# HarrisonKramer/optiland

Hardware: AMD Instinct MI355X
Metric: ray-surface intersections/s (higher is better)
Workload: dtype f32

## Files before the change

### optiland_amd/csrc/trace_kernel.hip

```cpp
#include <hip/hip_runtime.h>
#include <stdint.h>
#include <math.h>
#include <stdlib.h>

#include <type_traits>

#include "device_table.h"
#include "raygen_device.h"
#include "wavefront_device.h"
#include "epilogue_device.h"
#include "trace_launch.h"

#ifndef OL_TABLE_IN_LDS
#define OL_TABLE_IN_LDS 0
#endif
#ifndef OL_NR_PREFETCH
#define OL_NR_PREFETCH 0
#endif
#ifndef OL_PREFETCH_F64
#define OL_PREFETCH_F64 1
#endif
#ifndef OL_FUSED_NR_PREFETCH
#define OL_FUSED_NR_PREFETCH 1
#endif
#ifndef OL_FETCH_NR_F32
#define OL_FETCH_NR_F32 0
#endif
#ifndef OL_FETCH_NR_F32_PLAIN
#define OL_FETCH_NR_F32_PLAIN 1
#endif
#ifndef OL_FETCH_NR_F64
#define OL_FETCH_NR_F64 2
#endif
#ifndef OL_FETCH_NR_F64_ASPHERE
#define OL_FETCH_NR_F64_ASPHERE 1
#endif
#ifndef OL_FETCH_LEAN_F64
#define OL_FETCH_LEAN_F64 1
#endif
#ifndef OL_FETCH_LEAN_F32
#define OL_FETCH_LEAN_F32 1
#endif

#include "surface_math.h"

namespace ol {

template <typename T, int NR, bool FUSED, int POLK = 0>
constexpr int fetch_level() {
  if (OL_TABLE_IN_LDS) return 0;
  if (NR != 0) {
    if (sizeof(T) == 4) return (!FUSED && POLK == 0) ? OL_FETCH_NR_F32_PLAIN : OL_FETCH_NR_F32;
    return NR == kNrEvenAsphere ? OL_FETCH_NR_F64_ASPHERE : OL_FETCH_NR_F64;
  }
  if (!FUSED) return 0;
  return sizeof(T) == 4 ? OL_FETCH_LEAN_F32 : OL_FETCH_LEAN_F64;
}

template <typename T, int RPT, int POLK, int NR>
struct LanePack {
#ifndef OL_PACKED_F32
#define OL_PACKED_F32 1
#endif
#ifndef OL_POLZ_PACKED
#define OL_POLZ_PACKED 1
#endif
  static constexpr bool packed =
      sizeof(T) == 4 && ((OL_PACKED_F32 && (RPT == 4 || RPT == 2) && POLK == 0 && NR == 0) ||
                         (OL_POLZ_PACKED && RPT == 2 && POLK == 1 && NR == kNrZernike));
  using V = typename std::conditional<packed, f32x2, T>::type;
  static constexpr int NV = packed ? RPT / 2 : RPT;
  using PT = typename PrtLane<V, POLK>::type;
  using PrtArr = Prt<PT, POLK>[POLK ? NV : 1];
  static __device__ __forceinline__ T pget(const PrtArr& P, int k, int e) {
    if constexpr (packed && POLK != 0) return P[k / 2].m[e][k % 2]; else return P[k].m[e];
  }
  static __device__ __forceinline__ void pset(PrtArr& P, int k, int e, T x) {
    if constexpr (packed && POLK != 0) P[k / 2].m[e][k % 2] = x; else P[k].m[e] = x;
  }
  static __device__ __forceinline__ T get(const V& v, int e) {
    if constexpr (packed) return v[e]; else return v;
  }
  static __device__ __forceinline__ void set(V& v, int e, T x) {
    if constexpr (packed) v[e] = x; else v = x;
  }
  static __device__ __forceinline__ Ray<T> ray(const Ray<V> (&r)[NV], int k) {
    constexpr int L = packed ? 2 : 1;
    const Ray<V>& p = r[k / L];
    const int e = k % L;
    Ray<T> o;
    o.x = get(p.x, e); o.y = get(p.y, e); o.z = get(p.z, e);
    o.L = get(p.L, e); o.M = get(p.M, e); o.N = get(p.N, e);
    o.i = get(p.i, e); o.opd = get(p.opd, e);
    return o;
  }
  static __device__ __forceinline__ void put(Ray<V> (&r)[NV], int k, const Ray<T>& o) {
    constexpr int L = packed ? 2 : 1;
    Ray<V>& p = r[k / L];
    const int e = k % L;
    set(p.x, e, o.x); set(p.y, e, o.y); set(p.z, e, o.z);
    set(p.L, e, o.L); set(p.M, e, o.M); set(p.N, e, o.N);
    set(p.i, e, o.i); set(p.opd, e, o.opd);
  }
};

#ifndef OL_NT_SCALAR
#define OL_NT_SCALAR 1
#endif
#ifndef OL_NT_VECTOR
#define OL_NT_VECTOR 0
#endif

template <typename T, int RPT>
struct VecOf {
  typedef T type __attribute__((ext_vector_type(RPT)));
};

template <typename T, int RPT>
__device__ __forceinline__ T vec_get(const typename VecOf<T, RPT>::type& v, int k) {
  return v[k];
}

#ifndef OL_SADDR
#define OL_SADDR 1
#endif
#ifndef OL_RECORD_DIRECT
#define OL_RECORD_DIRECT 0
#endif
#ifndef OL_RECORD_ARGS_FRESH
#define OL_RECORD_ARGS_FRESH 1
#endif
#ifndef OL_PRT_SCALAR_BASE
#define OL_PRT_SCALAR_BASE 0
#endif
template <bool SADDR>
struct RayIndexT {
  int64_t tile;
  uint32_t lane;
  __device__ __forceinline__ int64_t full() const { return tile + (int64_t)lane; }
  template <typename P>
  __device__ __forceinline__ P* at(P* p) const {
    if constexpr (SADDR)
      return (p + tile) + lane;
    else
      return p + (tile + (int64_t)lane);
  }
};

template <typename T, int RPT, typename RayIndex>
__device__ __forceinline__ void store_plane(T* __restrict__ p, RayIndex base, int cnt,
                                            const T (&in)[RPT]) {
  T* q = base.at(p);
  if constexpr (RPT == 1) {
#if OL_NT_SCALAR
    __builtin_nontemporal_store(in[0], q);
#else
    *q = in[0];
#endif
  } else {
    using V = typename VecOf<T, RPT>::type;
    if (cnt == RPT) {
      V v;
#pragma unroll
      for (int k = 0; k < RPT; ++k) v[k] = in[k];
      if constexpr (OL_NT_VECTOR || sizeof(V) <= 8)
        __builtin_nontemporal_store(v, reinterpret_cast<V*>(q));
      else
        *reinterpret_cast<V*>(q) = v;
    } else {
#pragma unroll
      for (int k = 0; k < RPT; ++k)
        if (k < cnt) q[k] = in[k];
    }
  }
}

template <typename T, int RPT, typename RayIndex>
__device__ __forceinline__ void store_rays(T* __restrict__ row, int64_t stride, RayIndex base,
                                           int cnt, const Ray<T> (&g)[RPT]) {
  T tmp[RPT];
#define OL_STORE_FIELD(idx, fld)                         \
  _Pragma("unroll") for (int k = 0; k < RPT; ++k) tmp[k] = g[k].fld; \
  store_plane<T, RPT>(row + (int64_t)(idx) * stride, base, cnt, tmp);
  OL_STORE_FIELD(0, x)
  OL_STORE_FIELD(1, y)
  OL_STORE_FIELD(2, z)
  OL_STORE_FIELD(3, L)
  OL_STORE_FIELD(4, M)
  OL_STORE_FIELD(5, N)
  OL_STORE_FIELD(6, i)
  OL_STORE_FIELD(7, opd)
#undef OL_STORE_FIELD
}

__device__ __forceinline__ double spot_wave_sum(double v) {
#pragma unroll
  for (int off = 32; off > 0; off >>= 1) v += __shfl_down(v, off, 64);
  return v;
}
__device__ __forceinline__ double spot_wave_max(double v) {
#pragma unroll
  for (int off = 32; off > 0; off >>= 1) {
    const double o = __shfl_down(v, off, 64);
    v = o > v ? o : v;
  }
  return v;
}

struct SpotAcc {
  double s[6] = {0, 0, 0, 0, 0, 0};
  double rmax = 0.0;
  template <typename T>
  __device__ __forceinline__ void add(T x, T y, T i, double cx, double cy) {
    spot_accumulate<T>(s, rmax, x, y, i, cx, cy);
  }
  __device__ __forceinline__ void flush(double* __restrict__ out) {
    __shared__ double part[kTraceBlock / 64][7];
    const int lane = threadIdx.x & 63, wave = threadIdx.x >> 6;
    double v[7] = {s[0], s[1], s[2], s[3], s[4], s[5], rmax};
#pragma unroll
    for (int off = 32; off > 0; off >>= 1) {
      double o[7];
#pragma unroll
      for (int k = 0; k < 7; ++k) o[k] = __shfl_down(v[k], off, 64);
#pragma unroll
      for (int k = 0; k < 6; ++k) v[k] += o[k];
      v[6] = o[6] > v[6] ? o[6] : v[6];
    }
    if (lane == 0) {
#pragma unroll
      for (int k = 0; k < 7; ++k) part[wave][k] = v[k];
    }
    __builtin_amdgcn_fence(__ATOMIC_RELEASE, "workgroup", "local");
    __builtin_amdgcn_s_barrier();
    __builtin_amdgcn_fence(__ATOMIC_ACQUIRE, "workgroup", "local");
    if (threadIdx.x < 6) {
      double v = 0;
      for (int w = 0; w < kTraceBlock / 64; ++w) v += part[w][threadIdx.x];
      if (v != 0.0) unsafeAtomicAdd(&out[threadIdx.x], v);
    } else if (threadIdx.x == 6) {
      double v = part[0][6];
      for (int w = 1; w < kTraceBlock / 64; ++w) v = part[w][6] > v ? part[w][6] : v;
      if (v > 0.0)
        atomicMax(reinterpret_cast<unsigned long long*>(&out[6]),
                  (unsigned long long)__double_as_longlong(v));
    }
  }
};

#ifndef OL_POLNR_WAVES
#define OL_POLNR_WAVES 7
#endif

constexpr int kTraceArgsKernargOffset = 32;

template <typename A>
__device__ __forceinline__ cptr<A> kernarg_again(int offset) {
#if defined(__HIP_DEVICE_COMPILE__)
  using CP = const __attribute__((address_space(4))) char*;
  CP p = (CP)__builtin_amdgcn_kernarg_segment_ptr();
  asm volatile("" : "+s"(p));
  return reinterpret_cast<cptr<A>>(p + offset);
#else
  return nullptr;
#endif
}

template <typename T, typename A>
struct KernArgs {
  const DevSurfHot<T>* surf;
  const DevSurfCold<T>* cold;
  const DevOptics<T>* optics;
  const T* coeffs;
  A a;
};
template <typename T, typename A>
__device__ __forceinline__ cptr<KernArgs<T, A>> kernargs() {
  using KA = KernArgs<T, A>;
  static_assert(__builtin_offsetof(KA, a) == kTraceArgsKernargOffset, "kernarg layout");
  return kernarg_again<KernArgs<T, A>>(0);
}
template <bool FETCH, typename T, typename A>
__device__ __forceinline__ auto arg_view(const A& a) {
  if constexpr (FETCH) return &kernargs<T, A>()->a;
  else return &a;
}
template <typename C>
__device__ __forceinline__ C consts_of(const C* p) { return *p; }
#if defined(__HIP_DEVICE_COMPILE__)
template <typename C>
__device__ __forceinline__ C consts_of(cptr<C> p) { return load_consts(p); }
#endif
template <typename T, typename A>
__device__ __forceinline__ SurfFetched<T> fetched_surface(int s) {
  const auto ka = kernargs<T, A>();
  return SurfFetched<T>{as_const(ka->surf) + s, as_const(ka->cold) + s,
                        as_const(ka->optics) + (s * ka->a.n_wl + ka->a.wl)};
}
template <typename T, typename A>
__device__ __forceinline__ SurfFetched<T> fetched_surface_of(int s, const DevOptics<T>* optics,
                                                             int n_wl, int wl) {
  const auto ka = kernargs<T, A>();
  return SurfFetched<T>{as_const(ka->surf) + s, as_const(ka->cold) + s,
                        as_const(optics) + (s * n_wl + wl)};
}
#ifndef OL_POLNR_WAVES_F64
#define OL_POLNR_WAVES_F64 0
#endif
#ifndef OL_LEAN_F64_WAVES
#define OL_LEAN_F64_WAVES 0
#endif
#ifndef OL_POLZ_PAIR_WAVES
#define OL_POLZ_PAIR_WAVES 0
#endif
template <typename T, int RPT, int POLK, int NR, bool GEN = false>
struct WavesPerEu {
  static constexpr int value =
      (OL_POLZ_PAIR_WAVES > 0 && sizeof(T) == 4 && RPT == 2 && POLK == 1 && NR == kNrZernike)
          ? OL_POLZ_PAIR_WAVES
      : (OL_POLNR_WAVES > 0 && sizeof(T) == 4 && RPT == 1 && POLK == 1 && NR != 0 &&
       NR != kNrReference && !(GEN && NR == 1))
          ? OL_POLNR_WAVES
          : ((OL_POLNR_WAVES_F64 > 0 && sizeof(T) == 8 && RPT == 1 && POLK == 1 && NR != 0)
                 ? OL_POLNR_WAVES_F64
                 : ((OL_LEAN_F64_WAVES > 0 && sizeof(T) == 8 && RPT == 1 && POLK == 0 && NR == 0)
                        ? OL_LEAN_F64_WAVES
                        : 1));
};

template <typename T, int RPT = 1>
__device__ __forceinline__ T (*epi_launch_slots())[kTraceBlock * RPT] {
  __shared__ T slots[4][kTraceBlock * RPT];
  return slots;
}

template <typename T, int RPT, bool RECORD, int POLK, int NR, bool SPOT, int GEN = 0,
          bool EPI = false>
__global__ __launch_bounds__(kTraceBlock)
__attribute__((amdgpu_waves_per_eu(WavesPerEu<T, RPT, POLK, NR, GEN != 0 || EPI>::value))) void trace_kernel(
    const DevSurfHot<T>* __restrict__ surf_tab, const DevSurfCold<T>* __restrict__ cold_tab,
    const DevOptics<T>* __restrict__ optics_tab, const T* __restrict__ coeff_tab,
    TraceArgs<T> a) {
#if OL_TABLE_IN_LDS
  constexpr int kMaxLdsSurf = 64;
  __shared__ DevSurfHot<T> lds_hot[kMaxLdsSurf];
  __shared__ DevOptics<T> lds_opt[kMaxLdsSurf];
  {
    const int ns = a.last - a.first + 1;
    constexpr int HW = sizeof(DevSurfHot<T>) / 4, OW = sizeof(DevOptics<T>) / 4;
    const uint32_t* gh = reinterpret_cast<const uint32_t*>(surf_tab + a.first);
    uint32_t* lh = reinterpret_cast<uint32_t*>(lds_hot);
    for (int i = threadIdx.x; i < ns * HW; i += kTraceBlock) lh[i] = gh[i];
    uint32_t* lo = reinterpret_cast<uint32_t*>(lds_opt);
    for (int i = threadIdx.x; i < ns * OW; i += kTraceBlock) {
      const int sidx = i / OW, w = i % OW;
      lo[i] = reinterpret_cast<const uint32_t*>(optics_tab + (a.first + sidx) * a.n_wl + a.wl)[w];
    }
    __syncthreads();
  }
#endif
  using RayIndex = RayIndexT<(OL_SADDR != 0) && POLK != 0>;
  RayIndex base{(int64_t)blockIdx.x * (kTraceBlock * RPT), (uint32_t)threadIdx.x * RPT};
  const bool live = base.full() < a.n;
  if constexpr (!SPOT) {
    if (!live) return;
  } else if (RPT == 1 && !live) {
    base.lane = (uint32_t)(a.n - 1 - base.tile);
  }
  const int64_t left = a.n - base.full();
  const int cnt = RPT == 1 ? 1 : (left >= RPT ? RPT : (left > 0 ? (int)left : 0));

  using LP = LanePack<T, RPT, POLK, NR>;
  using V = typename LP::V;
  constexpr int NV = LP::NV;
  Ray<V> r[NV];
  constexpr int NPRT = POLK == 2 ? 18 : 9;
  typename LP::PrtArr P;
  uint32_t status = 0;
  if constexpr (GEN != 0) {
    static_assert(RPT == 1 || (RPT == 2 && GEN == kGenUniform && sizeof(T) == 4 &&
                               ((POLK == 0 && NR == 0) || (POLK == 1 && NR == kNrZernike))),
                  "the generating prologue: one ray per lane, the lean fp32 pair, or the "
                  "polarised Zernike fp32 pair (OL_POLZ_PAIR)");
    static_assert(GEN == kGenUniform || POLK == 0,
                  "polarised launches: the run-time general form (GEN == kGenUniform)");
    constexpr bool kGeneral = POLK != 0;
    const auto A0 = arg_view<(fetch_level<T, NR, false, POLK>() >= 1), T>(a);
    const auto& in_ = A0->in;
    T tx = in_.tx0, ty = in_.ty0, vx = in_.vx0, vy = in_.vy0, o[6];
    const RaygenConsts<T> c = consts_of(&A0->rgc);
    if constexpr ((GEN & kGenFieldPlanes) != 0 || kGeneral) {
      if (!kGeneral || in_.hx != nullptr) {
        const T hx = base.at(in_.hx)[0], hy = base.at(in_.hy)[0];
        if (in_.vx != nullptr) {
          vx = base.at(in_.vx)[0];
          vy = base.at(in_.vy)[0];
        }
        if ((in_.flags & kRaygenCheckField) && (outside_unit(hx) || outside_unit(hy)))
          status |= kStatusFieldRange;
        raygen_field<T>(c, hx, hy, tx, ty);
      }
    }
    T txs[RPT], tys[RPT], vxs[RPT], vys[RPT];
#pragma unroll
    for (int k = 0; k < RPT; ++k) {
      txs[k] = tx; tys[k] = ty; vxs[k] = vx; vys[k] = vy;
    }
    if constexpr (RPT > 1 && kGeneral) {
      if (in_.hx != nullptr) {
#pragma unroll
        for (int k = 1; k < RPT; ++k) {
          const int j = k < cnt ? k : 0;
          const T hx = base.at(in_.hx)[j], hy = base.at(in_.hy)[j];
          vxs[k] = in_.vx0;
          vys[k] = in_.vy0;
          if (in_.vx != nullptr) {
            vxs[k] = base.at(in_.vx)[j];
            vys[k] = base.at(in_.vy)[j];
          }
          if (k < cnt && (in_.flags & kRaygenCheckField) && (outside_unit(hx) || outside_unit(hy)))
            status |= kStatusFieldRange;
          txs[k] = in_.tx0;
          tys[k] = in_.ty0;
          raygen_field<T>(c, hx, hy, txs[k], tys[k]);
        }
      }
    }
    T pxs[RPT], pys[RPT];
    if constexpr (RPT == 1) {
      pxs[0] = base.at(in_.px)[0];
      pys[0] = base.at(in_.py)[0];
    } else if (cnt == RPT) {
      using PV = typename VecOf<T, RPT>::type;
      const PV vx_ = *reinterpret_cast<const PV*>(base.at(in_.px));
      const PV vy_ = *reinterpret_cast<const PV*>(base.at(in_.py));
#pragma unroll
      for (int k = 0; k < RPT; ++k) {
        pxs[k] = vec_get<T, RPT>(vx_, k);
        pys[k] = vec_get<T, RPT>(vy_, k);
      }
    } else {
#pragma unroll
      for (int k = 0; k < RPT; ++k) {
        pxs[k] = k < cnt ? base.at(in_.px)[k] : T(0);
        pys[k] = k < cnt ? base.at(in_.py)[k] : T(0);
      }
    }
#pragma unroll
    for (int k = 0; k < RPT; ++k) {
      T px = pxs[k], py = pys[k];
      uint32_t st_k = 0;
      raygen_pupil<T>(in_.flags, vxs[k], vys[k], px, py, st_k);
      if (k < cnt) status |= st_k;
      raygen_one<T>(c, txs[k], tys[k], px, py, vxs[k], vys[k], o);
      Ray<T> q;
      q.x = o[0]; q.y = o[1]; q.z = o[2];
      q.L = o[3]; q.M = o[4]; q.N = o[5];
      if constexpr ((GEN & kGenApod) != 0 || kGeneral) q.i = raygen_apodize<T>(c, px, py);
      else q.i = T(1);
      q.opd = T(0);
      LP::put(r, k, q);
      if constexpr (EPI) {
        T (*epi_launch)[kTraceBlock * RPT] = epi_launch_slots<T, RPT>();
        epi_launch[0][threadIdx.x * RPT + k] = q.L;
        epi_launch[1][threadIdx.x * RPT + k] = q.M;
        epi_launch[2][threadIdx.x * RPT + k] = q.N;
        epi_launch[3][threadIdx.x * RPT + k] = q.i;
      }
    }
    if constexpr (POLK != 0) {
#pragma unroll
      for (int k = 0; k < RPT; ++k)
#pragma unroll
        for (int e = 0; e < NPRT; ++e) LP::pset(P, k, e, (e == 0 || e == 4 || e == 8) ? T(1) : T(0));
    }
  } else
  {
    T in[8][RPT];
    T pin[POLK ? NPRT : 1][RPT];
    if (RPT > 1 && cnt == RPT) {
      using V = typename VecOf<T, RPT>::type;
      V v[8];
#pragma unroll
      for (int f = 0; f < 8; ++f) v[f] = *reinterpret_cast<const V*>(base.at(a.rays[f]));
      if constexpr (POLK != 0) {
        if (!(a.flags & kTracePrtIdentity)) {
          V pv[NPRT];
#pragma unroll
          for (int e = 0; e < NPRT; ++e)
            pv[e] = *reinterpret_cast<const V*>(base.at(a.prt + (int64_t)e * a.n));
#pragma unroll
          for (int e = 0; e < NPRT; ++e)
#pragma unroll
            for (int k = 0; k < RPT; ++k) pin[e][k] = vec_get<T, RPT>(pv[e], k);
        }
      }
#pragma unroll
      for (int f = 0; f < 8; ++f)
#pragma unroll
        for (int k = 0; k < RPT; ++k) in[f][k] = vec_get<T, RPT>(v[f], k);
    } else {
#pragma unroll
      for (int f = 0; f < 8; ++f)
#pragma unroll
        for (int k = 0; k < RPT; ++k) in[f][k] = k < cnt ? base.at(a.rays[f])[k] : T(0);
      if constexpr (POLK != 0) {
        if (!(a.flags & kTracePrtIdentity)) {
#pragma unroll
          for (int e = 0; e < NPRT; ++e)
#pragma unroll
            for (int k = 0; k < RPT; ++k)
              pin[e][k] = k < cnt ? base.at(a.prt + (int64_t)e * a.n)[k] : T(0);
        }
      }
    }
#pragma unroll
    for (int k = 0; k < RPT; ++k) {
      Ray<T> o;
      o.x = in[0][k]; o.y = in[1][k]; o.z = in[2][k];
      o.L = in[3][k]; o.M = in[4][k]; o.N = in[5][k];
      o.i = in[6][k]; o.opd = in[7][k];
      LP::put(r, k, o);
      if constexpr (POLK != 0) {
        const bool ident = (a.flags & kTracePrtIdentity) != 0;
#pragma unroll
        for (int e = 0; e < NPRT; ++e)
          LP::pset(P, k, e, ident ? ((e == 0 || e == 4 || e == 8) ? T(1) : T(0)) : pin[e][k]);
      }
    }
  }

  bool is_global = true;
  bool prt_fresh = POLK != 0 && (GEN != 0 || (a.flags & kTracePrtIdentity) != 0);
  constexpr bool kFetch = fetch_level<T, NR, false, POLK>() >= 2;
  constexpr bool kFetchArgs = fetch_level<T, NR, false, POLK>() >= 1;
  const cptr<T> coeffs_c = as_const(coeff_tab);
  constexpr bool kShareRcp = !RECORD && RPT > 1;
  DevSurf<T> last_traced;
  last_traced.cold = as_const(cold_tab);
  int last_idx = a.first;
  auto to_global_now = [&](Ray<V> (&gv)[NV]) {
    if constexpr (kFetch) {
      const DevSurf<T> lt = fetched_surface<T, TraceArgs<T>>(last_idx).surf();
#pragma unroll
      for (int j = 0; j < NV; ++j) gv[j] = is_global ? r[j] : to_global<V>(lt, r[j]);
    } else {
#pragma unroll
      for (int j = 0; j < NV; ++j) gv[j] = is_global ? r[j] : to_global<V>(last_traced, r[j]);
    }
  };
#if OL_TABLE_IN_LDS
// ... 166 lines not shown
  }
  if ((late.flags & kTraceWriteRays) && (!SPOT || live)) {
    Ray<V> gv[NV];
    to_global_now(gv);
    Ray<T> g[RPT];
#pragma unroll
    for (int k = 0; k < RPT; ++k) g[k] = LP::ray(gv, k);
    T tmp[RPT];
#define OL_WB_FIELD(idx, fld)                                        \
  _Pragma("unroll") for (int k = 0; k < RPT; ++k) tmp[k] = g[k].fld; \
  store_plane<T, RPT>(late.rays[idx], base, cnt, tmp);
    OL_WB_FIELD(0, x)
    OL_WB_FIELD(1, y)
    OL_WB_FIELD(2, z)
    OL_WB_FIELD(3, L)
    OL_WB_FIELD(4, M)
    OL_WB_FIELD(5, N)
    OL_WB_FIELD(6, i)
    OL_WB_FIELD(7, opd)
#undef OL_WB_FIELD
  }
  if constexpr (POLK != 0) {
    T tmp[RPT];
#pragma unroll
    for (int e = 0; e < NPRT; ++e) {
#pragma unroll
      for (int k = 0; k < RPT; ++k) tmp[k] = LP::pget(P, k, e);
      T* plane = late.prt + (int64_t)e * late.n;
#if OL_PRT_SCALAR_BASE
      plane = refresh(plane);
#endif
      store_plane<T, RPT>(plane, base, cnt, tmp);
    }
  }
  if constexpr (EPI) {
    static_assert(GEN == kGenUniform && POLK != 0,
                  "the update_intensity epilogue: generating polarised launches");
    const auto ka = kernargs<T, TraceArgs<T>>();
    T* upd = ka->a.i_updated;
    {
      PolFields<T> f;
#pragma unroll
      for (int k = 0; k < 2; ++k) {
        f.ar[k] = ka->a.pf.ar[k]; f.ai[k] = ka->a.pf.ai[k];
        f.br[k] = ka->a.pf.br[k]; f.bi[k] = ka->a.pf.bi[k];
      }
      f.nf = ka->a.pf.nf;
      T (*epi_launch)[kTraceBlock * RPT] = epi_launch_slots<T, RPT>();
      T upd_k[RPT];
#pragma unroll
      for (int k = 0; k < RPT; ++k) {
        T Pm[9], Qm[9];
#pragma unroll
        for (int e = 0; e < 9; ++e) {
          Pm[e] = LP::pget(P, k, e);
          Qm[e] = POLK == 2 ? LP::pget(P, k, POLK == 2 ? 9 + e : e) : T(0);
        }
        const int slot = threadIdx.x * RPT + k;
        const T L0 = epi_launch[0][slot], M0 = epi_launch[1][slot], N0 = epi_launch[2][slot],
                i0 = epi_launch[3][slot];
        uint32_t st_k = 0;
        upd_k[k] = pol_intensity_one<T, POLK == 2>(f, L0, M0, N0, Pm, Qm, i0, st_k);
        if (k < cnt) status |= st_k;
      }
      if constexpr (RPT == 1) base.at(upd)[0] = upd_k[0];
      else store_plane<T, RPT>(upd, base, cnt, upd_k);
    }
  }
  if (status && late.status) atomicOr(late.status, status);
}

template <typename T>
static unsigned record_lds(const TraceArgs<T>& a, bool lean, bool generating) {
  if (a.record == nullptr) return 0;
  int cap = tuning().record_wg_cap;
  if (cap == 0)
    cap = !lean ? 1 : sizeof(T) == 8 ? 3 : !(a.flags & kTraceFewWaves) ? 1 : generating ? 2 : 3;
  if (cap < 2) return 0;
  const unsigned want = 160u * 1024u / (unsigned)cap - 1024u;
  return want > 63u * 1024u ? 63u * 1024u : want;
}

template <typename T, int RPT, int NR>
static hipError_t launch_nr(const TraceArgs<T>& a, hipStream_t stream) {
  const int64_t threads = (a.n + RPT - 1) / RPT;
  const int64_t blocks = (threads + kTraceBlock - 1) / kTraceBlock;
  if (blocks == 0) return hipSuccess;
  if (blocks > 0x7fffffffLL) return hipErrorInvalidValue;
  dim3 grid((unsigned)blocks), block(kTraceBlock);
  const bool rec = a.record != nullptr;
  const int polk = a.prt == nullptr ? 0 : ((a.flags & kTracePrtComplex) ? 2 : 1);
#define OL_LAUNCH_S(R, P, S)                                                                 \
  hipLaunchKernelGGL((trace_kernel<T, RPT, R, P, NR, S>), grid, block,                        \
                     record_lds(a, NR == 0 && P == 0, false), stream, a.surf, a.cold,         \
                     a.optics, a.coeffs, a)
#define OL_LAUNCH(R, P) OL_LAUNCH_S(R, P, false)
  if (a.spot != nullptr) {
    if (polk != 0 || NR == kNrReference) return hipErrorInvalidValue;
    if constexpr (NR != kNrReference) {
      if (rec) OL_LAUNCH_S(true, 0, true); else OL_LAUNCH_S(false, 0, true);
    }
    return hipGetLastError();
  }
  if (polk == 2) {
    if constexpr (RPT == 1) {
      if (rec) OL_LAUNCH(true, 2); else OL_LAUNCH(false, 2);
    } else {
      return hipErrorInvalidValue;
    }
  } else if (rec && polk == 1) OL_LAUNCH(true, 1);
  else if (rec) OL_LAUNCH(true, 0);
  else if (polk == 1) OL_LAUNCH(false, 1);
  else OL_LAUNCH(false, 0);
#undef OL_LAUNCH_S
#undef OL_LAUNCH
  return hipGetLastError();
}

template <typename T, int RPT>
static hipError_t launch_rpt(const TraceArgs<T>& a, int nr, hipStream_t stream) {
  if (nr == 0) return launch_nr<T, RPT, 0>(a, stream);
  if constexpr (RPT > 1) {
    if (nr == 2) return launch_nr<T, RPT, 2>(a, stream);
  } else {
    if (a.spot == nullptr) {
      if (nr == kNrZernike) return launch_nr<T, 1, kNrZernike>(a, stream);
      if (nr == kNrEvenAsphere) return launch_nr<T, 1, kNrEvenAsphere>(a, stream);
    }
    if (nr == kNrReference) return launch_nr<T, 1, kNrReference>(a, stream);
  }
  return launch_nr<T, RPT, 1>(a, stream);
}

template <typename T>
static hipError_t launch_pair(const TraceArgs<T>& a, hipStream_t stream) {
  const int64_t threads = (a.n + 1) / 2;
  const int64_t blocks = (threads + kTraceBlock - 1) / kTraceBlock;
  if (blocks == 0) return hipSuccess;
  if (blocks > 0x7fffffffLL) return hipErrorInvalidValue;
  dim3 grid((unsigned)blocks), block(kTraceBlock);
  if (a.record != nullptr)
    hipLaunchKernelGGL((trace_kernel<T, 2, true, 0, 0, false>), grid, block,
                       record_lds(a, true, false), stream, a.surf, a.cold, a.optics, a.coeffs,
                       a);
  else
    hipLaunchKernelGGL((trace_kernel<T, 2, false, 0, 0, false>), grid, block, 0, stream, a.surf,
                       a.cold, a.optics, a.coeffs, a);
  return hipGetLastError();
}

#ifndef OL_GEN_PAIR
#define OL_GEN_PAIR 1
#endif
template <typename T>
static hipError_t launch_gen_pair(const TraceArgs<T>& a, hipStream_t stream) {
  const int64_t threads = (a.n + 1) / 2;
  const int64_t blocks = (threads + kTraceBlock - 1) / kTraceBlock;
  if (blocks == 0) return hipSuccess;
  if (blocks > 0x7fffffffLL) return hipErrorInvalidValue;
  const dim3 grid((unsigned)blocks), block(kTraceBlock);
  if (a.spot != nullptr)
    hipLaunchKernelGGL((trace_kernel<T, 2, true, 0, 0, true, kGenUniform, false>), grid, block,
                       record_lds(a, true, true), stream, a.surf, a.cold, a.optics, a.coeffs, a);
  else
    hipLaunchKernelGGL((trace_kernel<T, 2, true, 0, 0, false, kGenUniform, false>), grid, block,
                       record_lds(a, true, true), stream, a.surf, a.cold, a.optics, a.coeffs, a);
  return hipGetLastError();
}

template <typename T, int NR>
static hipError_t launch_gen_nr(const TraceArgs<T>& a, bool pair_ok, hipStream_t stream) {
  if constexpr (sizeof(T) == 4 && NR == 0) {
    const int want = tuning().rays_per_thread;
    if (pair_ok && a.prt == nullptr && a.in.hx == nullptr && a.rgc.apod_kind == 0 &&
        (want == 3 || (want == 0 && OL_GEN_PAIR)))
      return launch_gen_pair<T>(a, stream);
  }
  if constexpr (sizeof(T) == 4 && NR == kNrZernike) {
    const int want = tuning().rays_per_thread;
    if (pair_ok && a.prt != nullptr && !(a.flags & kTracePrtComplex) && a.spot == nullptr &&
        a.n % 2 == 0 && reinterpret_cast<uintptr_t>(a.prt) % 8 == 0 &&
        reinterpret_cast<uintptr_t>(a.i_updated) % 8 == 0 &&
        (want == 3 || (want == 0 && OL_POLZ_PAIR))) {
      const int64_t threads = (a.n + 1) / 2;
      const int64_t blocks2 = (threads + kTraceBlock - 1) / kTraceBlock;
      if (blocks2 == 0) return hipSuccess;
      if (blocks2 > 0x7fffffffLL) return hipErrorInvalidValue;
      const dim3 grid2((unsigned)blocks2), block2(kTraceBlock);
      if (a.i_updated != nullptr)
        hipLaunchKernelGGL((trace_kernel<T, 2, true, 1, NR, false, kGenUniform, true>), grid2,
                           block2, 0, stream, a.surf, a.cold, a.optics, a.coeffs, a);
      else
        hipLaunchKernelGGL((trace_kernel<T, 2, true, 1, NR, false, kGenUniform, false>), grid2,
                           block2, 0, stream, a.surf, a.cold, a.optics, a.coeffs, a);
      return hipGetLastError();
    }
  }
  const int64_t blocks = (a.n + kTraceBlock - 1) / kTraceBlock;
  if (blocks == 0) return hipSuccess;
  if (blocks > 0x7fffffffLL) return hipErrorInvalidValue;
  dim3 grid((unsigned)blocks), block(kTraceBlock);
  const int polk = a.prt == nullptr ? 0 : ((a.flags & kTracePrtComplex) ? 2 : 1);
#define OL_LAUNCH_G(P, S, G, E)                                                              \
  hipLaunchKernelGGL((trace_kernel<T, 1, true, P, NR, S, G, E>), grid, block,                 \
                     record_lds(a, NR == 0 && P == 0, G == kGenUniform), stream, a.surf,     \
                     a.cold, a.optics, a.coeffs, a)
  const bool epi = polk != 0 && a.i_updated != nullptr;
  const bool fieldp = a.in.hx != nullptr, apod = a.rgc.apod_kind != 0;
  if (polk != 0) {
    if (a.spot != nullptr) return hipErrorInvalidValue;
    if (polk == 2) { if (epi) OL_LAUNCH_G(2, false, 1, true); else OL_LAUNCH_G(2, false, 1, false); }
    else { if (epi) OL_LAUNCH_G(1, false, 1, true); else OL_LAUNCH_G(1, false, 1, false); }
  } else if (a.spot != nullptr) {
    if (fieldp || apod) return hipErrorInvalidValue;
    OL_LAUNCH_G(0, true, 1, false);
  } else {
    if (fieldp && apod) OL_LAUNCH_G(0, false, 7, false);
    else if (fieldp) OL_LAUNCH_G(0, false, 3, false);
    else if (apod) OL_LAUNCH_G(0, false, 5, false);
    else OL_LAUNCH_G(0, false, 1, false);
  }
#undef OL_LAUNCH_G
  return hipGetLastError();
}

template <typename T>
hipError_t launch_trace_generate(const TraceArgs<T>& a_in, int nr_family, bool pair_ok,
                                 hipStream_t stream) {
  TraceArgs<T> a = a_in;
  if (nr_family == kNrReference) return hipErrorInvalidValue;
  if (nr_family == kNrNone) return launch_gen_nr<T, 0>(a, pair_ok, stream);
  if (nr_family == kNrZernike) return launch_gen_nr<T, kNrZernike>(a, pair_ok, stream);
  if (nr_family == kNrEvenAsphere) return launch_gen_nr<T, kNrEvenAsphere>(a, false, stream);
  return launch_gen_nr<T, 1>(a, false, stream);
}

#if OL_TRACE_TU == 0 || OL_TRACE_TU == 1
Tuning& tuning() {
  static Tuning t = [] {
    Tuning v;
    if (const char* e = getenv("OL_TRACE_RPT")) v.rays_per_thread = atoi(e);
    if (const char* e = getenv("OL_RECORD_WG_CAP")) {
      const int c = atoi(e);
      if (c >= 0 && c <= 8) v.record_wg_cap = c;
    }
    return v;
  }();
  return t;
}
#endif

template <typename T>
hipError_t launch_trace(const TraceArgs<T>& a, bool vector_ok, int nr_family,
                        hipStream_t stream) {
  constexpr int kVec = 16 / sizeof(T);
  const int nr = nr_family == kNrNone
                     ? kNrNone
                     : ((a.flags & kTraceCompact) && tuning().compact ? kNrCompact : nr_family);
  if (nr_family == kNrReference) {
    if (a.nr_iters == nullptr) return hipErrorInvalidValue;
    return launch_rpt<T, 1>(a, kNrReference, stream);
  }
  if (!vector_ok || (a.prt && (a.flags & kTracePrtComplex)))
    return launch_rpt<T, 1>(a, nr == 2 ? 1 : nr, stream);
  const int want = tuning().rays_per_thread;
  if constexpr (sizeof(T) == 4) {
    if (want == 3 && nr == 0 && a.prt == nullptr && a.spot == nullptr)
      return launch_pair<T>(a, stream);
  }
  const bool prefer_one = (nr != kNrNone && nr != kNrCompact) || a.record != nullptr;
  if (want == 1 || (want == 0 && prefer_one && nr != 2))
    return launch_rpt<T, 1>(a, nr == 2 ? 1 : nr, stream);
  return launch_rpt<T, kVec>(a, nr, stream);
}

#ifndef OL_TRACE_TU
#define OL_TRACE_TU 0
#endif
#if OL_TRACE_TU == 0 || OL_TRACE_TU == 1
template hipError_t launch_trace<float>(const TraceArgs<float>&, bool, int, hipStream_t);
template hipError_t launch_trace_generate<float>(const TraceArgs<float>&, int, bool,
                                                 hipStream_t);
#endif
#if OL_TRACE_TU == 0 || OL_TRACE_TU == 2
template hipError_t launch_trace<double>(const TraceArgs<double>&, bool, int, hipStream_t);
template hipError_t launch_trace_generate<double>(const TraceArgs<double>&, int, bool,
                                                  hipStream_t);
#endif


struct NoBatch {
  char unused;
};
template <typename T, int RPT, int NR, bool FIELDP, bool APOD, bool BATCH = false>
__global__ __launch_bounds__(kTraceBlock) void spot_trace_kernel(
    const DevSurfHot<T>* __restrict__ surf_tab, const DevSurfCold<T>* __restrict__ cold_tab,
    const DevOptics<T>* __restrict__ optics_tab, const T* __restrict__ coeff_tab,
    SpotArgs<T> a, typename std::conditional<BATCH, SpotBatch<T>, NoBatch>::type batch) {
  static_assert(!(BATCH && FIELDP), "a batched cell has ONE field point");
  constexpr bool kFetch = fetch_level<T, NR, true>() >= 1;
  constexpr bool kFetchRows = fetch_level<T, NR, true>() >= 2;
  constexpr bool field_planes = FIELDP;

  SpotAcc acc;
  uint32_t status = 0;
  bool prt_fresh = false;
  constexpr int64_t kTileRays = (int64_t)kTraceBlock * RPT;
  const int tiles_per_block = a.tiles_per_block;

  for (int tt = 0; tt < tiles_per_block; ++tt) {
    const auto A0 = arg_view<kFetch, T>(a);
    const int64_t n_rays = A0->n;
    const int64_t ntiles = (n_rays + kTileRays - 1) / kTileRays;
    const int64_t tile = (int64_t)blockIdx.x * tiles_per_block + tt;
    if (tile >= ntiles) break;
    const int64_t base = (tile * kTraceBlock + threadIdx.x) * RPT;
    const int64_t left = n_rays - base;
    const int cnt = left >= RPT ? RPT : (left > 0 ? (int)left : 0);
    const auto& in_ = A0->in;
    const bool vig_planes = !BATCH && in_.vx != nullptr;
    T tx0, ty0, vx0, vy0;
    if constexpr (BATCH) {
      const SpotCell<T>& cell = batch.c[blockIdx.y];
      tx0 = cell.tx; ty0 = cell.ty; vx0 = cell.vx; vy0 = cell.vy;
    } else {
      tx0 = in_.tx0; ty0 = in_.ty0; vx0 = in_.vx0; vy0 = in_.vy0;
    }
    const uint32_t rg_flags = in_.flags;

    T in[6][RPT];
    if (RPT > 1 && cnt == RPT) {
      using V = typename VecOf<T, RPT>::type;
      V v[6];
      v[0] = *reinterpret_cast<const V*>(in_.px + base);
      v[1] = *reinterpret_cast<const V*>(in_.py + base);
      if constexpr (FIELDP) {
        v[2] = *reinterpret_cast<const V*>(in_.hx + base);
        v[3] = *reinterpret_cast<const V*>(in_.hy + base);
      }
      if (vig_planes) {
        v[4] = *reinterpret_cast<const V*>(in_.vx + base);
        v[5] = *reinterpret_cast<const V*>(in_.vy + base);
      }
#pragma unroll
      for (int k = 0; k < RPT; ++k) {
        in[0][k] = vec_get<T, RPT>(v[0], k);
        in[1][k] = vec_get<T, RPT>(v[1], k);
        in[2][k] = field_planes ? vec_get<T, RPT>(v[2], k) : T(0);
        in[3][k] = field_planes ? vec_get<T, RPT>(v[3], k) : T(0);
        in[4][k] = vig_planes ? vec_get<T, RPT>(v[4], k) : vx0;
        in[5][k] = vig_planes ? vec_get<T, RPT>(v[5], k) : vy0;
      }
    } else {
#pragma unroll
      for (int k = 0; k < RPT; ++k) {
        const bool ok = k < cnt;
        in[0][k] = ok ? in_.px[base + k] : T(0);
        in[1][k] = ok ? in_.py[base + k] : T(0);
        in[2][k] = (ok && field_planes) ? in_.hx[base + k] : T(0);
        in[3][k] = (ok && field_planes) ? in_.hy[base + k] : T(0);
        in[4][k] = (ok && vig_planes) ? in_.vx[base + k] : vx0;
        in[5][k] = (ok && vig_planes) ? in_.vy[base + k] : vy0;
      }
    }

    using LP = LanePack<T, RPT, 0, NR>;
    using V = typename LP::V;
    constexpr int NV = LP::NV;
    Ray<V> r[NV];
    {
      const RaygenConsts<T> c = consts_of(&A0->rgc);
#pragma unroll
      for (int k = 0; k < RPT; ++k) {
        T tx = tx0, ty = ty0, o[6];
        if constexpr (FIELDP) {
          if ((rg_flags & kRaygenCheckField) && (outside_unit(in[2][k]) || outside_unit(in[3][k])))
            status |= kStatusFieldRange;
          raygen_field<T>(c, in[2][k], in[3][k], tx, ty);
        }
        raygen_pupil<T>(rg_flags, in[4][k], in[5][k], in[0][k], in[1][k], status);
        raygen_one<T>(c, tx, ty, in[0][k], in[1][k], in[4][k], in[5][k], o);
        Ray<T> q;
        q.x = o[0]; q.y = o[1]; q.z = o[2];
        q.L = o[3]; q.M = o[4]; q.N = o[5];
        if constexpr (APOD) q.i = raygen_apodize<T>(c, in[0][k], in[1][k]); else q.i = T(1);
        q.opd = T(0);
        LP::put(r, k, q);
      }
    }

    bool is_global = true;
    DevSurf<T> last_traced;
    last_traced.cold = as_const(cold_tab);
    Prt<T, 0> P[1];
    Ray<V> gv[NV];
    if constexpr (kFetchRows) {
      int last_idx = 0;
      const int first = kernargs<T, SpotArgs<T>>()->a.first;
      for (int s = first; s <= kernargs<T, SpotArgs<T>>()->a.last; ++s) {
        const SurfFetched<T> h = [&](int s_) {
          if constexpr (BATCH)
            return fetched_surface_of<T, SpotArgs<T>>(s_, batch.c[blockIdx.y].optics,
                                                      batch.c[blockIdx.y].n_wl,
                                                      batch.c[blockIdx.y].wl);
          else
            return fetched_surface<T, SpotArgs<T>>(s_);
        }(s);
        if (refresh(h.hot)->interaction != kRecordOnly) {
          surface_step<V, NV, 0, NR, (RPT > 1)>(h, as_const(kernargs<T, SpotArgs<T>>()->coeffs), is_global, r,
                                     P, status, prt_fresh);
          is_global = false;
          last_idx = s;
        }
      }
      const DevSurf<T> lt = fetched_surface<T, SpotArgs<T>>(last_idx).surf();
      const bool keep =
          is_global || (kernargs<T, SpotArgs<T>>()->a.in.flags & kSpotHitsLocal) != 0;
#pragma unroll
      for (int j = 0; j < NV; ++j) gv[j] = keep ? r[j] : to_global<V>(lt, r[j]);
    } else {
      constexpr bool kPrefetch =
          (OL_FUSED_NR_PREFETCH || NR == 0) && (OL_PREFETCH_F64 || sizeof(T) == 4);
      DevSurfHot<T> cur = surf_tab[a.first];
      for (int s = a.first; s <= a.last; ++s) {
        DevSurf<T> S;
        if constexpr (kPrefetch) {
          static_cast<DevSurfHot<T>&>(S) = cur;
          if (s < a.last) cur = surf_tab[s + 1];
        } else {
          static_cast<DevSurfHot<T>&>(S) = surf_tab[s];
        }
        S.cold = as_const(cold_tab) + s;
        if (S.interaction != kRecordOnly) {
          DevOptics<T> O;
          if constexpr (BATCH) {
            const SpotCell<T>& cell = batch.c[blockIdx.y];
            O = cell.optics[s * cell.n_wl + cell.wl];
          } else {
            O = optics_tab[s * a.n_wl + a.wl];
          }
          surface_step<V, NV, 0, NR, (RPT > 1)>(S, O, as_const(coeff_tab), is_global, r, P, status,
                                     prt_fresh);
          is_global = false;
          last_traced = S;
        }
      }
      const bool keep = is_global || (a.in.flags & kSpotHitsLocal) != 0;
#pragma unroll
      for (int j = 0; j < NV; ++j) gv[j] = keep ? r[j] : to_global<V>(last_traced, r[j]);
    }

    T hx_[RPT], hy_[RPT], hi_[RPT];
    const auto A1 = arg_view<kFetch, T>(a);
    double cx, cy;
    if constexpr (BATCH) {
      cx = batch.c[blockIdx.y].cx; cy = batch.c[blockIdx.y].cy;
    } else {
      cx = A1->cx; cy = A1->cy;
    }
#pragma unroll
    for (int k = 0; k < RPT; ++k) {
      const Ray<T> g = LP::ray(gv, k);
      hx_[k] = g.x; hy_[k] = g.y; hi_[k] = g.i;
      if (k < cnt) acc.add(g.x, g.y, g.i, cx, cy);
    }
    if (A1->hits[0] != nullptr && cnt > 0) {
      const RayIndexT<false> at{tile * (kTraceBlock * RPT), (uint32_t)threadIdx.x * RPT};
      int64_t cell_off = 0;
      if constexpr (BATCH) cell_off = (int64_t)blockIdx.y * 3 * batch.hits_stride;
      store_plane<T, RPT>(A1->hits[0] + cell_off, at, cnt, hx_);
      store_plane<T, RPT>(A1->hits[1] + cell_off, at, cnt, hy_);
      store_plane<T, RPT>(A1->hits[2] + cell_off, at, cnt, hi_);
    }
  }

  const auto A2 = arg_view<kFetch, T>(a);
  if constexpr (BATCH) acc.flush(A2->out + 8 * blockIdx.y);
  else acc.flush(A2->out);
  uint32_t* status_out = A2->status;
  if (status && status_out) atomicOr(status_out, status);
}

template <typename T, int RPT, int NR, bool BATCH = false>
static hipError_t launch_spot_nr(const SpotArgs<T>& a_in, hipStream_t stream,
                                 const SpotBatch<T>* batch = nullptr) {
  SpotArgs<T> a = a_in;
  const int64_t tile_rays = (int64_t)kTraceBlock * RPT;
  const int64_t ntiles = (a.n + tile_rays - 1) / tile_rays;
  static const int forced = [] {
    const char* e = getenv("OL_SPOT_TILES");
    return e ? atoi(e) : 0;
  }();
  constexpr int64_t kTargetBlocks = 8192;
  const int64_t cells = BATCH ? batch->n_cells : 1;
  int64_t tpb = forced > 0 ? forced : (ntiles * cells + kTargetBlocks - 1) / kTargetBlocks;
  if (tpb < 1) tpb = 1;
  if (tpb > 1024) tpb = 1024;
  a.tiles_per_block = (int32_t)tpb;
  a.rgc = RaygenConsts<T>(a.rg);
  if (!BATCH && a.in.hx == nullptr) uniform_field_tangents<T>(a.rg, a.in);
  const int64_t blocks = (ntiles + tpb - 1) / tpb;
  if (blocks == 0 || cells == 0) return hipSuccess;
  if (blocks > 0x7fffffffLL) return hipErrorInvalidValue;
  const bool apod = a.rg.apod_kind != 0;
  if constexpr (BATCH) {
#define OL_SPOT_LAUNCH_B(A)                                                                   \
  hipLaunchKernelGGL((spot_trace_kernel<T, RPT, NR, false, A, true>),                         \
                     dim3((unsigned)blocks, (unsigned)cells), dim3(kTraceBlock), 0, stream,   \
                     a.surf, a.cold, a.optics, a.coeffs, a, *batch)
    if (apod) OL_SPOT_LAUNCH_B(true);
    else OL_SPOT_LAUNCH_B(false);
#undef OL_SPOT_LAUNCH_B
  } else {
#define OL_SPOT_LAUNCH(F, A)                                                               \
  hipLaunchKernelGGL((spot_trace_kernel<T, RPT, NR, F, A>), dim3((unsigned)blocks),        \
                     dim3(kTraceBlock), 0, stream, a.surf, a.cold, a.optics, a.coeffs, a,  \
                     NoBatch{})
    const bool fieldp = a.in.hx != nullptr;
    if (fieldp && apod) OL_SPOT_LAUNCH(true, true);
    else if (fieldp) OL_SPOT_LAUNCH(true, false);
    else if (apod) OL_SPOT_LAUNCH(false, true);
    else OL_SPOT_LAUNCH(false, false);
#undef OL_SPOT_LAUNCH
  }
  return hipGetLastError();
}

template <typename T, bool BATCH>
static hipError_t dispatch_spot(const SpotArgs<T>& a, const SpotBatch<T>* batch, bool vector_ok,
                                int nr_family, hipStream_t stream) {
  constexpr int kVec = 16 / sizeof(T);
  const int want = tuning().rays_per_thread;
  if (nr_family != kNrNone) {
    if (vector_ok && want == 2) return launch_spot_nr<T, kVec, 1, BATCH>(a, stream, batch);
    if (nr_family == kNrZernike) return launch_spot_nr<T, 1, kNrZernike, BATCH>(a, stream, batch);
    if (nr_family == kNrEvenAsphere)
      return launch_spot_nr<T, 1, kNrEvenAsphere, BATCH>(a, stream, batch);
    return launch_spot_nr<T, 1, 1, BATCH>(a, stream, batch);
  }
  if (!vector_ok || want == 1) return launch_spot_nr<T, 1, 0, BATCH>(a, stream, batch);
  return launch_spot_nr<T, kVec, 0, BATCH>(a, stream, batch);
}

template <typename T>
hipError_t launch_spot_trace(const SpotArgs<T>& a, bool vector_ok, int nr_family,
                             hipStream_t stream) {
  return dispatch_spot<T, false>(a, nullptr, vector_ok, nr_family, stream);
}

template <typename T>
hipError_t launch_spot_batch(const SpotArgs<T>& a, const SpotBatch<T>& batch, bool vector_ok,
                             int nr_family, hipStream_t stream) {
  if (batch.n_cells < 0 || batch.n_cells > kSpotBatchCells) return hipErrorInvalidValue;
  return dispatch_spot<T, true>(a, &batch, vector_ok, nr_family, stream);
}

#if OL_TRACE_TU == 0 || OL_TRACE_TU == 1
template hipError_t launch_spot_trace<float>(const SpotArgs<float>&, bool, int, hipStream_t);
template hipError_t launch_spot_batch<float>(const SpotArgs<float>&, const SpotBatch<float>&, bool,
                                             int, hipStream_t);
#endif
#if OL_TRACE_TU == 0 || OL_TRACE_TU == 2
template hipError_t launch_spot_trace<double>(const SpotArgs<double>&, bool, int, hipStream_t);
template hipError_t launch_spot_batch<double>(const SpotArgs<double>&, const SpotBatch<double>&,
                                              bool, int, hipStream_t);
#endif

template <typename T, int NR, bool APOD, bool DEVREF = false, int RPT = 1>
__global__ __launch_bounds__(kTraceBlock) void opd_trace_kernel(
    const DevSurfHot<T>* __restrict__ surf_tab, const DevSurfCold<T>* __restrict__ cold_tab,
    const DevOptics<T>* __restrict__ optics_tab, const T* __restrict__ coeff_tab,
    OpdArgs<T> a) {
  constexpr bool kFetch = fetch_level<T, NR, true>() >= 1;
  constexpr bool kFetchRows = fetch_level<T, NR, true>() >= 2;
  uint32_t status = 0;
  bool prt_fresh = false;
  double s[kOpdMoments];
#pragma unroll
  for (int k = 0; k < kOpdMoments; ++k) s[k] = 0.0;

  for (int64_t j = ((int64_t)blockIdx.x * kTraceBlock + threadIdx.x) * RPT;
       j < arg_view<kFetch, T>(a)->n; j += (int64_t)gridDim.x * kTraceBlock * RPT) {
    Ray<T> r[RPT];
    int cnt = RPT;
    {
      const auto A0 = arg_view<kFetch, T>(a);
      const auto& in_ = A0->in;
      T px[RPT], py[RPT];
      if constexpr (RPT == 1) {
        px[0] = in_.px[j]; py[0] = in_.py[j];
      } else {
        const int64_t left = A0->n - j;
        cnt = left >= RPT ? RPT : (int)left;
        if (cnt == RPT) {
          using PV = typename VecOf<T, RPT>::type;
          const PV vx_ = *reinterpret_cast<const PV*>(in_.px + j);
          const PV vy_ = *reinterpret_cast<const PV*>(in_.py + j);
#pragma unroll
          for (int k = 0; k < RPT; ++k) {
            px[k] = vec_get<T, RPT>(vx_, k); py[k] = vec_get<T, RPT>(vy_, k);
          }
        } else {
#pragma unroll
          for (int k = 0; k < RPT; ++k) {
            px[k] = k < cnt ? in_.px[j + k] : T(0); py[k] = k < cnt ? in_.py[j + k] : T(0);
          }
        }
      }
      const RaygenConsts<T> c = consts_of(&A0->rgc);
#pragma unroll
      for (int k = 0; k < RPT; ++k) {
        T vx = in_.vx0, vy = in_.vy0, o[6];
        uint32_t st = 0;
        raygen_pupil<T>(in_.flags, vx, vy, px[k], py[k], st);
        if (k < cnt) status |= st;
        raygen_one<T>(c, in_.tx0, in_.ty0, px[k], py[k], vx, vy, o);
        r[k].x = o[0]; r[k].y = o[1]; r[k].z = o[2];
        r[k].L = o[3]; r[k].M = o[4]; r[k].N = o[5];
        if constexpr (APOD) r[k].i = raygen_apodize<T>(c, px[k], py[k]); else r[k].i = T(1);
        r[k].opd = T(0);
      }
    }

    bool is_global = true;
    DevSurf<T> last_traced;
    last_traced.cold = as_const(cold_tab);
    Prt<T, 0> P[1];
    Ray<T> g[RPT];
    if constexpr (kFetchRows) {
      int last_idx = 0;
      const int first = kernargs<T, OpdArgs<T>>()->a.first;
      for (int sidx = first; sidx <= kernargs<T, OpdArgs<T>>()->a.last; ++sidx) {
        const SurfFetched<T> h = fetched_surface<T, OpdArgs<T>>(sidx);
        if (refresh(h.hot)->interaction != kRecordOnly) {
          surface_step<T, RPT, 0, NR>(h, as_const(kernargs<T, OpdArgs<T>>()->coeffs), is_global,
                                      r, P, status, prt_fresh);
          is_global = false;
          last_idx = sidx;
        }
      }
      const DevSurf<T> lt = fetched_surface<T, OpdArgs<T>>(last_idx).surf();
#pragma unroll
      for (int k = 0; k < RPT; ++k) g[k] = is_global ? r[k] : to_global<T>(lt, r[k]);
    } else {
      constexpr bool kPrefetch =
          (OL_FUSED_NR_PREFETCH || NR == 0) && (OL_PREFETCH_F64 || sizeof(T) == 4);
      DevSurfHot<T> cur = surf_tab[a.first];
      for (int sidx = a.first; sidx <= a.last; ++sidx) {
        DevSurf<T> S;
        if constexpr (kPrefetch) {
          static_cast<DevSurfHot<T>&>(S) = cur;
          if (sidx < a.last) cur = surf_tab[sidx + 1];
        } else {
          static_cast<DevSurfHot<T>&>(S) = surf_tab[sidx];
        }
        S.cold = as_const(cold_tab) + sidx;
        if (S.interaction != kRecordOnly) {
          const DevOptics<T> O = optics_tab[sidx * a.n_wl + a.wl];
          surface_step<T, RPT, 0, NR>(S, O, as_const(coeff_tab), is_global, r, P, status,
                                      prt_fresh);
          is_global = false;
          last_traced = S;
        }
      }
#pragma unroll
      for (int k = 0; k < RPT; ++k) g[k] = is_global ? r[k] : to_global<T>(last_traced, r[k]);
    }
    const auto A1 = arg_view<kFetch, T>(a);
    T ov[RPT], gi[RPT], pu[3][RPT];
    {
      WavefrontConsts<T> w;
      if constexpr (DEVREF) w = load_consts(as_const(A1->wf_dev));
      else w = consts_of(&A1->wfc);
#pragma unroll
      for (int k = 0; k < RPT; ++k) {
        final_propagate<T, false>(w, g[k]);
        const int64_t jk = k < cnt ? j + k : j;
        T q[3];
        ov[k] = wavefront_one<T>(w, g[k].x, g[k].y, g[k].z, g[k].L, g[k].M, g[k].N, g[k].opd,
                                 A1->in.px[jk], A1->in.py[jk], q);
        gi[k] = g[k].i;
        pu[0][k] = q[0]; pu[1][k] = q[1]; pu[2][k] = q[2];
      }
    }
    T* const pup0 = A1->pupil[0];
    if constexpr (RPT == 1) {
      A1->opd[j] = ov[0];
      A1->inten[j] = gi[0];
      if (pup0) {
        pup0[j] = pu[0][0];
        A1->pupil[1][j] = pu[1][0];
        A1->pupil[2][j] = pu[2][0];
      }
    } else {
      const RayIndexT<false> at{j, 0u};
      store_plane<T, RPT>(A1->opd, at, cnt, ov);
      store_plane<T, RPT>(A1->inten, at, cnt, gi);
      if (pup0) {
        store_plane<T, RPT>(pup0, at, cnt, pu[0]);
        store_plane<T, RPT>(A1->pupil[1], at, cnt, pu[1]);
        store_plane<T, RPT>(A1->pupil[2], at, cnt, pu[2]);
      }
    }
#pragma unroll
    for (int k = 0; k < RPT; ++k)
      if (k < cnt)
        opd_accumulate(s, (double)gi[k], (double)ov[k], (double)pu[0][k], (double)pu[1][k],
                       gi[k] > T(0));
  }

  __shared__ double part[kTraceBlock / 64][kOpdMoments];
  const int lane = threadIdx.x & 63, wave = threadIdx.x >> 6;
#pragma unroll
  for (int off = 32; off > 0; off >>= 1) {
    double t[kOpdMoments];
#pragma unroll
    for (int k = 0; k < kOpdMoments; ++k) t[k] = __shfl_down(s[k], off, 64);
#pragma unroll
    for (int k = 0; k < kOpdMoments; ++k) s[k] += t[k];
  }
  if (lane == 0) {
#pragma unroll
    for (int k = 0; k < kOpdMoments; ++k) part[wave][k] = s[k];
  }
  __syncthreads();
  if (threadIdx.x < kOpdMoments) {
    double v = 0;
    for (int q = 0; q < kTraceBlock / 64; ++q) v += part[q][threadIdx.x];
    if (v != 0.0) unsafeAtomicAdd(&arg_view<kFetch, T>(a)->mom[threadIdx.x], v);
  }
  uint32_t* status_out = arg_view<kFetch, T>(a)->status;
  if (status && status_out) atomicOr(status_out, status);
}

template <typename T>
hipError_t launch_opd_trace(const OpdArgs<T>& a_in, bool vector_ok, int nr_family,
                            hipStream_t stream) {
  OpdArgs<T> a = a_in;
  uniform_field_tangents<T>(a.rg, a.in);
  a.rgc = RaygenConsts<T>(a.rg);
  a.wfc = WavefrontConsts<T>(a.wf);
  if (a.n == 0) return hipSuccess;
#ifndef OL_OPD_TWO_RAYS
#define OL_OPD_TWO_RAYS 1
#endif
  const bool two = OL_OPD_TWO_RAYS && vector_ok && nr_family == kNrNone &&
                   tuning().rays_per_thread != 1 && a.n >= (int64_t)4096 * kTraceBlock;
  const int64_t per_block = (int64_t)kTraceBlock * (two ? 2 : 1);
  int64_t blocks = (a.n + per_block - 1) / per_block;
  if (blocks > 8192) blocks = 8192;
  const bool apod = a.rg.apod_kind != 0;
#define OL_OPD_LAUNCH_R(N, A, R)                                                             \
  do {                                                                                       \
    if (a.wf_dev != nullptr)                                                                 \
      hipLaunchKernelGGL((opd_trace_kernel<T, N, A, true, R>), dim3((unsigned)blocks),       \
                         dim3(kTraceBlock), 0, stream, a.surf, a.cold, a.optics, a.coeffs, a); \
    else                                                                                     \
      hipLaunchKernelGGL((opd_trace_kernel<T, N, A, false, R>), dim3((unsigned)blocks),      \
                         dim3(kTraceBlock), 0, stream, a.surf, a.cold, a.optics, a.coeffs, a); \
  } while (0)
#define OL_OPD_LAUNCH(N, A) OL_OPD_LAUNCH_R(N, A, 1)
  if (nr_family == kNrZernike) {
    if (apod) OL_OPD_LAUNCH(kNrZernike, true); else OL_OPD_LAUNCH(kNrZernike, false);
  } else if (nr_family == kNrEvenAsphere) {
    if (apod) OL_OPD_LAUNCH(kNrEvenAsphere, true); else OL_OPD_LAUNCH(kNrEvenAsphere, false);
  } else if (nr_family != kNrNone) {
    if (apod) OL_OPD_LAUNCH(1, true); else OL_OPD_LAUNCH(1, false);
  } else if (two) {
    if (apod) OL_OPD_LAUNCH_R(0, true, 2); else OL_OPD_LAUNCH_R(0, false, 2);
  } else {
    if (apod) OL_OPD_LAUNCH(0, true); else OL_OPD_LAUNCH(0, false);
  }
#undef OL_OPD_LAUNCH
#undef OL_OPD_LAUNCH_R
  return hipGetLastError();
}

#if OL_TRACE_TU == 0 || OL_TRACE_TU == 2
template hipError_t launch_opd_trace<double>(const OpdArgs<double>&, bool, int, hipStream_t);
#endif

template <typename T, int NR>
__global__ __launch_bounds__(64) void chief_ref_kernel(
    const DevSurfHot<T>* __restrict__ surf_tab, const DevSurfCold<T>* __restrict__ cold_tab,
    const DevOptics<T>* __restrict__ optics_tab, const T* __restrict__ coeff_tab,
    ChiefArgs<T> a) {
  if (threadIdx.x != 0 || blockIdx.x != 0) return;
  using m = Math<T>;
  uint32_t status = 0;
  bool prt_fresh = false;
  Ray<T> r[1];
  {
    T px = T(0), py = T(0), vx = a.in.vx0, vy = a.in.vy0, o[6];
    raygen_pupil<T>(a.in.flags, vx, vy, px, py, status);
    raygen_one<T>(a.rgc, a.in.tx0, a.in.ty0, px, py, vx, vy, o);
    r[0].x = o[0]; r[0].y = o[1]; r[0].z = o[2];
    r[0].L = o[3]; r[0].M = o[4]; r[0].N = o[5];
    r[0].i = T(1);
    r[0].opd = T(0);
  }
  bool is_global = true;
  int last_idx = a.first;
  Prt<T, 0> P[1];
  for (int s = a.first; s <= a.last; ++s) {
    const SurfFetched<T> h{as_const(surf_tab) + s, as_const(cold_tab) + s,
                           as_const(optics_tab) + (s * a.n_wl + a.wl)};
    if (refresh(h.hot)->interaction != kRecordOnly) {
      surface_step<T, 1, 0, NR>(h, as_const(coeff_tab), is_global, r, P, status, prt_fresh);
      is_global = false;
      last_idx = s;
    }
  }
  Ray<T> g = r[0];
  if (!is_global) {
    const SurfFetched<T> h{as_const(surf_tab) + last_idx, as_const(cold_tab) + last_idx,
                           as_const(optics_tab) + (last_idx * a.n_wl + a.wl)};
    g = to_global<T>(h.surf(), r[0]);
  }
  WavefrontConsts<T> w = a.wfc;
  final_propagate<T, true>(w, g);
  w.xc = g.x; w.yc = g.y; w.zc = g.z;
  T t_back;
  if (w.planar) {
    w.R = T(0);
    w.nx = g.L; w.ny = g.M; w.nz = g.N;
    t_back = T(0);
  } else {
    const T dz = g.z - a.pupil_z;
    w.R = m::sqrt(g.x * g.x + g.y * g.y + dz * dz);
    w.nx = w.ny = w.nz = T(0);
    const T aa = g.L * g.L + g.M * g.M + g.N * g.N;
    const T d = T(4) * aa * w.R * w.R;
    const T sq = m::sqrt(d < T(0) ? T(0) : d);
    const T t1 = m::div(-sq, T(2) * aa), t2 = m::div(sq, T(2) * aa);
    t_back = t1 < T(0) ? t2 : t1;
  }
  w.opd_ref = g.opd - w.ni * t_back;
  *a.out = w;
  if (a.chief != nullptr) {
    a.chief[0] = g.x; a.chief[1] = g.y; a.chief[2] = g.z; a.chief[3] = g.L;
    a.chief[4] = g.M; a.chief[5] = g.N; a.chief[6] = g.i; a.chief[7] = g.opd;
  }
  if (status && a.status) atomicOr(a.status, status);
}

template <typename T>
hipError_t launch_chief_reference(const ChiefArgs<T>& a_in, int nr_family, hipStream_t stream) {
  ChiefArgs<T> a = a_in;
  uniform_field_tangents<T>(a.rg, a.in);
  a.rgc = RaygenConsts<T>(a.rg);
#define OL_CHIEF_LAUNCH(N)                                                                   \
  hipLaunchKernelGGL((chief_ref_kernel<T, N>), dim3(1), dim3(64), 0, stream, a.surf, a.cold, \
                     a.optics, a.coeffs, a)
  if (nr_family == kNrNone) OL_CHIEF_LAUNCH(0);
  else OL_CHIEF_LAUNCH(1);
#undef OL_CHIEF_LAUNCH
  return hipGetLastError();
}
#if OL_TRACE_TU == 0 || OL_TRACE_TU == 2
template hipError_t launch_chief_reference<double>(const ChiefArgs<double>&, int, hipStream_t);
#endif

}
```

Before: 206.2 billion.

## Park per-thread double accumulators in LDS and set waves-per-EU hints for OPD

The spot and OPD kernels keep their f64 running sums in per-thread LDS slots across the tile loop instead of in registers. Each iteration reloads them, accumulates, and stores them back. This frees VGPRs during the expensive trace section. The OPD kernel also gets amdgpu_waves_per_eu occupancy hints for the no-NR and Zernike variants. The cost is extra LDS traffic per tile, plus a larger LDS footprint (7 or kOpdMoments doubles per thread) that may limit occupancy.

New measurement: 207.3 billion (median of 5 runs). No clear change (+0.5%).

```diff
diff --git a/optiland_amd/csrc/trace_kernel.hip b/optiland_amd/csrc/trace_kernel.hip
--- a/optiland_amd/csrc/trace_kernel.hip
+++ b/optiland_amd/csrc/trace_kernel.hip
@@ -247,6 +247,30 @@
     }
   }
 };
+
+template <int N>
+__device__ __forceinline__ void fetch_sums(const double (&slot)[N][kTraceBlock], double (&v)[N]) {
+#pragma unroll
+  for (int k = 0; k < N; ++k) v[k] = slot[k][threadIdx.x];
+}
+template <int N>
+__device__ __forceinline__ void park_sums(double (&slot)[N][kTraceBlock], const double (&v)[N]) {
+#pragma unroll
+  for (int k = 0; k < N; ++k) slot[k][threadIdx.x] = v[k];
+}
+__device__ __forceinline__ SpotAcc fetch_spot(const double (&slot)[7][kTraceBlock]) {
+  double v[7];
+  fetch_sums(slot, v);
+  SpotAcc acc;
+#pragma unroll
+  for (int k = 0; k < 6; ++k) acc.s[k] = v[k];
+  acc.rmax = v[6];
+  return acc;
+}
+__device__ __forceinline__ void park_spot(double (&slot)[7][kTraceBlock], const SpotAcc& acc) {
+  const double v[7] = {acc.s[0], acc.s[1], acc.s[2], acc.s[3], acc.s[4], acc.s[5], acc.rmax};
+  park_sums(slot, v);
+}
 
 #ifndef OL_POLNR_WAVES
 #define OL_POLNR_WAVES 7
@@ -1019,7 +1043,8 @@
   constexpr bool kFetchRows = fetch_level<T, NR, true>() >= 2;
   constexpr bool field_planes = FIELDP;
 
-  SpotAcc acc;
+  __shared__ double sums[7][kTraceBlock];
+  park_spot(sums, SpotAcc{});
   uint32_t status = 0;
   bool prt_fresh = false;
   constexpr int64_t kTileRays = (int64_t)kTraceBlock * RPT;
@@ -1175,12 +1200,14 @@
     } else {
       cx = A1->cx; cy = A1->cy;
     }
+    SpotAcc acc = fetch_spot(sums);
 #pragma unroll
     for (int k = 0; k < RPT; ++k) {
       const Ray<T> g = LP::ray(gv, k);
       hx_[k] = g.x; hy_[k] = g.y; hi_[k] = g.i;
       if (k < cnt) acc.add(g.x, g.y, g.i, cx, cy);
     }
+    park_spot(sums, acc);
     if (A1->hits[0] != nullptr && cnt > 0) {
       const RayIndexT<false> at{tile * (kTraceBlock * RPT), (uint32_t)threadIdx.x * RPT};
       int64_t cell_off = 0;
@@ -1192,6 +1219,7 @@
   }
 
   const auto A2 = arg_view<kFetch, T>(a);
+  SpotAcc acc = fetch_spot(sums);
   if constexpr (BATCH) acc.flush(A2->out + 8 * blockIdx.y);
   else acc.flush(A2->out);
   uint32_t* status_out = A2->status;
@@ -1283,8 +1311,19 @@
                                               bool, int, hipStream_t);
 #endif
 
+template <int NR>
+constexpr bool opd_sums_parked() { return NR == kNrNone || NR == kNrZernike; }
+template <int NR, int RPT, bool APOD>
+constexpr int opd_waves_per_eu() {
+  return APOD ? 1 : (NR == kNrNone && RPT == 2) ? 5 : (NR == kNrZernike ? 4 : 1);
+}
+__device__ __forceinline__ double (&opd_sum_slots())[kOpdMoments][kTraceBlock] {
+  __shared__ double slots[kOpdMoments][kTraceBlock];
+  return slots;
+}
 template <typename T, int NR, bool APOD, bool DEVREF = false, int RPT = 1>
-__global__ __launch_bounds__(kTraceBlock) void opd_trace_kernel(
+__global__ __launch_bounds__(kTraceBlock)
+__attribute__((amdgpu_waves_per_eu(opd_waves_per_eu<NR, RPT, APOD>()))) void opd_trace_kernel(
     const DevSurfHot<T>* __restrict__ surf_tab, const DevSurfCold<T>* __restrict__ cold_tab,
     const DevOptics<T>* __restrict__ optics_tab, const T* __restrict__ coeff_tab,
     OpdArgs<T> a) {
@@ -1292,9 +1331,11 @@
   constexpr bool kFetchRows = fetch_level<T, NR, true>() >= 2;
   uint32_t status = 0;
   bool prt_fresh = false;
+  constexpr bool kPark = opd_sums_parked<NR>();
   double s[kOpdMoments];
 #pragma unroll
   for (int k = 0; k < kOpdMoments; ++k) s[k] = 0.0;
+  if constexpr (kPark) park_sums(opd_sum_slots(), s);
 
   for (int64_t j = ((int64_t)blockIdx.x * kTraceBlock + threadIdx.x) * RPT;
        j < arg_view<kFetch, T>(a)->n; j += (int64_t)gridDim.x * kTraceBlock * RPT) {
@@ -1419,15 +1460,18 @@
         store_plane<T, RPT>(A1->pupil[2], at, cnt, pu[2]);
       }
     }
+    if constexpr (kPark) fetch_sums(opd_sum_slots(), s);
 #pragma unroll
     for (int k = 0; k < RPT; ++k)
       if (k < cnt)
         opd_accumulate(s, (double)gi[k], (double)ov[k], (double)pu[0][k], (double)pu[1][k],
                        gi[k] > T(0));
+    if constexpr (kPark) park_sums(opd_sum_slots(), s);
   }
 
   __shared__ double part[kTraceBlock / 64][kOpdMoments];
   const int lane = threadIdx.x & 63, wave = threadIdx.x >> 6;
+  if constexpr (kPark) fetch_sums(opd_sum_slots(), s);
 #pragma unroll
   for (int off = 32; off > 0; off >>= 1) {
     double t[kOpdMoments];
```
